# zjucsxxd/hdr2yuv

Hardware: AMD Instinct MI355X
Metric: Mpixels/s, 4K RGB->YUV420 PQ convert path (in-memory, HBM-resident) (higher is better)
Workload: dtype f32+f64

## Files before the change

### hdr2yuv_amd/api.py

```python
from __future__ import annotations

import ctypes as C
import os
import subprocess
from typing import Sequence

import numpy as np

_HERE = os.path.dirname(os.path.abspath(__file__))
_LIB = None

SAMPLE_U16, SAMPLE_F32, SAMPLE_F16 = 1, 2, 3
CHROMA_420, CHROMA_444 = 1, 3
TRANSFER_LINEAR, TRANSFER_PQ = 8, 16
MATRIX_GBR, MATRIX_BT709, MATRIX_BT2020NC, MATRIX_YDZDX, MATRIX_Y500, MATRIX_Y100 = 0, 1, 9, 11, 12, 13
MATRIX_YUVPRIME2 = 15
MATRIX_ICTCP = 14

H2Y_OK, H2Y_EINVAL, H2Y_EUNSUPPORTED, H2Y_EHIP, H2Y_ENOMEM = 0, 1, 2, 3, 4

EXPORTS = [
    "h2y_abi_version", "h2y_frame_bytes", "h2y_plane_bytes", "h2y_desc_check", "h2y_ctx_create", "h2y_ctx_destroy",
    "h2y_last_error", "h2y_ctx_set_stream", "h2y_convert_frame", "h2y_convert_batch", "h2y_convert_batch_enqueue",
    "h2y_batch_finish", "h2y_pic_stats", "h2y_matrix_convert", "h2y_subsample_420", "h2y_last_kernel_ms", "h2y_last_kernel_name", "h2y_last_kernel_variant",
    "h2y_matrix_inverse", "h2y_upsample_444", "h2y_inverse_420", "h2y_inverse_frame", "h2y_ctx_set_option", "h2y_stream_open", "h2y_stream_input", "h2y_stream_submit", "h2y_stream_output", "h2y_stream_close",
    "h2y_inverse_batch", "h2y_inverse_stream_open", "h2y_dpx_parse", "h2y_dpx_decode_batch", "h2y_dpx_stream_open",
    "h2y_tiff_parse", "h2y_tiff_layout", "h2y_tiff_decode_batch", "h2y_rgb_interleave_batch", "h2y_tiff_stream_open",
    "h2y_tiff_inverse_stream_open", "h2y_exr_parse", "h2y_exr_unpack", "h2y_exr_decode_batch", "h2y_exr_stream_open",
    "h2y_compare_batch", "h2y_stream_compare", "h2y_stream_reference", "h2y_stream_compare_result", "h2y_compare_stream_open",
    "h2y_histogram_batch", "h2y_stream_histogram", "h2y_stream_histogram_ex", "h2y_stream_histogram_result",
    "h2y_histogram_stream_open", "h2y_ssim_batch", "h2y_stream_ssim", "h2y_stream_ssim_result",
    "h2y_regions_host", "h2y_regions_batch", "h2y_stream_regions", "h2y_stream_regions_result",
    "h2y_light_batch", "h2y_stream_light", "h2y_stream_light_result",
    "h2y_lightdist_batch", "h2y_stream_lightdist", "h2y_stream_lightdist_result", "h2y_lightdist_json",
    "h2y_codelight_batch", "h2y_codelight_stream_open",
    "h2y_scenesig_batch", "h2y_codescenesig_batch", "h2y_stream_scenesig", "h2y_stream_scenesig_result", "h2y_stream_lightdist_bins",
    "h2y_scene_distance", "h2y_scene_cuts", "h2y_scene_merge", "h2y_lightdist_json_scenes",
    "h2y_linearize_batch", "h2y_pqcode_stream_open",
    "h2y_deltae_batch", "h2y_stream_deltae", "h2y_stream_deltae_result",
# ... 600 lines not shown
    L.h2y_stream_tonemap.argtypes = [C.c_void_p] + [C.c_int] * 3
    L.h2y_stream_tonemap.restype = C.c_int
    L.h2y_stream_open.argtypes = [C.c_void_p, C.POINTER(H2YDesc), C.c_int]
    L.h2y_stream_input.restype = C.c_int
    L.h2y_stream_input.argtypes = [C.c_void_p, C.POINTER(C.c_void_p)]
    L.h2y_stream_submit.restype = C.c_int
    L.h2y_stream_submit.argtypes = [C.c_void_p]
    L.h2y_stream_output.restype = C.c_int
    L.h2y_stream_output.argtypes = [C.c_void_p, C.POINTER(C.POINTER(C.c_uint16))]
    L.h2y_stream_close.restype = C.c_int
    L.h2y_stream_close.argtypes = [C.c_void_p]
    L.h2y_last_kernel_name.restype = C.c_char_p
    L.h2y_last_kernel_name.argtypes = [C.c_void_p]
    L.h2y_last_kernel_variant.restype = C.c_char_p
    L.h2y_last_kernel_variant.argtypes = [C.c_void_p]
    L.h2y_last_kernel_ms.restype = C.c_int
    L.h2y_last_kernel_ms.argtypes = [C.c_void_p, C.POINTER(C.c_float), C.POINTER(C.c_int)]
    _LIB = L
    return L


def frame_bytes(d: H2YDesc) -> int:
    return int(load_library().h2y_frame_bytes(C.byref(d)))


def desc_check(d: H2YDesc):
    why = C.c_char_p()
    rc = load_library().h2y_desc_check(C.byref(d), C.byref(why))
    return rc, (why.value or b"").decode()

# ... 1117 lines not shown
        self._stream_cmp_planes = None
        self._stream_out_words = None
        self._stream_pack_bytes = None
        self._stream_unpack_bytes = None
        self._stream_in_geom = None
        self._stream_out_geom = None
        self._stream_inverse = None
        self._stream_dpx = None
        self._stream_rgb = False

    def last_kernel_name(self) -> str:
        return (self.lib.h2y_last_kernel_name(self.h) or b"").decode()

    def last_kernel_variant(self) -> str:
        return (self.lib.h2y_last_kernel_variant(self.h) or b"").decode()
```

### hdr2yuv_amd/csrc/h2y_api.hip

```cpp
#include "h2y_shim.h"

#include <zlib.h>

static thread_local std::string g_err;

int fail(h2y_ctx *ctx, int code, const char *fmt, ...)
{
    char buf[512];
    va_list ap;
    va_start(ap, fmt);
    vsnprintf(buf, sizeof buf, fmt, ap);
    va_end(ap);
    g_err = buf;
    if (ctx) ctx->err = buf;
    return code;
}

int h2y_abi_version(void)
{
#ifdef H2Y_EXPERIMENT
    return H2Y_ABI_VERSION | H2Y_ABI_EXPERIMENT;
#else
    return H2Y_ABI_VERSION;
#endif
// ... 84 lines not shown
        HIP_TRY(ctx, hipEventCreateWithFlags(&b.ev_done, hipEventDisableTiming));
    }
    {
        std::vector<pq_recA> A(H2Y_PQ_NREC);
        std::vector<pq_recB> B(H2Y_PQ_NREC);
        pq_build_table(A.data(), B.data());
        HIP_TRY(ctx, hipMalloc(&ctx->d_table, H2Y_PQ_TABLE_BYTES));
        char *t = static_cast<char *>(ctx->d_table);
        HIP_TRY(ctx, hipMemcpy(t, A.data(), H2Y_PQ_NREC * 16, hipMemcpyHostToDevice));
        HIP_TRY(ctx, hipMemcpy(t + H2Y_PQ_NREC * 16, B.data(), H2Y_PQ_NREC * 16, hipMemcpyHostToDevice));
        {
            std::vector<pq_ext_rec> X(H2Y_PQX_NSEG);
            pq_build_table_ext(X.data());
            HIP_TRY(ctx, hipMalloc(&ctx->d_table_ext, H2Y_PQX_TABLE_BYTES));
            HIP_TRY(ctx, hipMemcpy(ctx->d_table_ext, X.data(), H2Y_PQX_TABLE_BYTES, hipMemcpyHostToDevice));
        }
        std::vector<pq_rec1> T1(H2Y_T1_NREC);
        pq_build_table1(T1.data());
        HIP_TRY(ctx, hipMalloc(&ctx->d_table1, H2Y_T1_NREC * sizeof(pq_rec1)));
        HIP_TRY(ctx, hipMemcpy(ctx->d_table1, T1.data(), H2Y_T1_NREC * sizeof(pq_rec1), hipMemcpyHostToDevice));
        HIP_TRY(ctx, hipMalloc((void **)&ctx->d_lut16, H2Y_LUT16_N * sizeof(float)));
        HIP_TRY(ctx, h2y_launch_build_lut16(ctx->stream, ctx->d_table, ctx->d_lut16));
        HIP_TRY(ctx, hipStreamSynchronize(ctx->stream));
    }
    for (batch_state &b : ctx->bs) {
        HIP_TRY(ctx, hipMalloc((void **)&b.d_assumed, 2 * sizeof(assumed_stats)));
        HIP_TRY(ctx, hipHostMalloc((void **)&b.h_assumed, 2 * sizeof(assumed_stats), hipHostMallocDefault));
        ctx->b = &b;
        const int rc = reserve_batch(ctx, 64);
        if (rc) return rc;
// ... 88 lines not shown
        (void)hipFree(b.d_partial);
        (void)hipFree(b.d_redo);
        (void)hipFree(b.d_low);
        (void)hipFree(b.d_clock);
        (void)hipHostFree(b.h_ranges);
        (void)hipHostFree(b.h_btime);
        (void)hipFree(b.d_tail);
        (void)hipFree(b.d_unit_rows);
        (void)hipHostFree(b.h_unit_rows);
        (void)hipFree(b.d_fstats);
        (void)hipHostFree(b.h_fstats);
        (void)hipFree(b.d_assumed);
        (void)hipHostFree(b.h_assumed);
    }
    (void)hipFree(ctx->d_table);
    for (void *t : ctx->d_tfn) (void)hipFree(t);
    for (int fn = 0; fn < H2Y_TFN_COUNT; fn++)
        if (ctx->d_tfn_ext[fn] && ctx->d_tfn_ext[fn] != ctx->d_table_ext) (void)hipFree(ctx->d_tfn_ext[fn]);
    (void)hipFree(ctx->d_lut16);
    (void)hipFree(ctx->d_table1);
    (void)hipFree(ctx->d_table_ext);
    (void)hipFree(ctx->d_tmp);
    (void)hipFree(ctx->d_lin);
    (void)hipFree(ctx->d_tab);
    (void)hipHostFree(ctx->h_tab);
    (void)hipFree(ctx->d_in);
    (void)hipFree(ctx->d_out);
    if (ctx->fir_stream) {
        (void)hipStreamSynchronize(ctx->fir_stream);
        (void)hipStreamDestroy(ctx->fir_stream);
// ... 1006 lines not shown
    case TIFF: return tiff_decode(ctx, tiff, clamp != 0, frames, n);
    case EXR: return exr_decode(ctx, exr, frames, n);
    default: return hipErrorInvalidValue;
    }
}

const char *decode_src::kernel() const { return kind == DPX ? "k_dpx_decode" : kind == TIFF ? "k_tiff_decode" : kind == EXR ? "k_exr_decode" : ""; }

std::string decode_src::variant() const
{
    return kind == DPX ? dpx_variant(dpx) : kind == TIFF ? tiff_variant(tiff, clamp != 0) : kind == EXR ? exr_variant(exr) : std::string();
}

const char *h2y_last_kernel_name(const h2y_ctx *ctx) { return ctx ? ctx->last_name : ""; }
const char *h2y_last_kernel_variant(const h2y_ctx *ctx) { return ctx ? ctx->last_variant.c_str() : ""; }

int h2y_last_kernel_ms(const h2y_ctx *ctx, float *ms, int *launches)
{
    if (!ctx) return H2Y_EINVAL;
    if (ms) *ms = ctx->last_ms;
    if (launches) *launches = ctx->last_launches;
    return H2Y_OK;
}
```

### hdr2yuv_amd/csrc/h2y_device.h

```cpp
#ifndef H2Y_DEVICE_H
#define H2Y_DEVICE_H

#include <hip/hip_runtime.h>
#include <stdint.h>

#include "h2y_kernels.h"
#include "h2y_math.h"

using namespace h2y;

#define WAVE 64

__device__ __forceinline__ float wave_min(float v)
{
#pragma unroll
    for (int o = 32; o > 0; o >>= 1) v = fminf(v, __shfl_xor(v, o, WAVE));
    return v;
}
__device__ __forceinline__ float wave_max(float v)
{
#pragma unroll
    for (int o = 32; o > 0; o >>= 1) v = fmaxf(v, __shfl_xor(v, o, WAVE));
    return v;
}
// ... 227 lines not shown
        const double d = pq_poly(xb, a, b);
        v = cand ? (float)d : v;
        slow = cand ? pq_ambiguous(d) : slow;
    }
    return v;
}

static __device__ __attribute__((noinline)) float tf_to_linear_careful(int cls, float v) { return tf_to_linear(cls, v); }
static __device__ __attribute__((noinline)) float tf_from_linear_careful(int cls, float v) { return tf_from_linear(cls, v); }

#define H2Y_PIPE_RUNTIME 0
#define H2Y_PIPE_PQ_IDENT 1
#define H2Y_PIPE_PQ_NORM 2
#define H2Y_PIPE_NONE 6
#define H2Y_PIPE_TFN 7

template <int PIPE> __device__ __forceinline__ float norm1(const pix_params &pp, int c, float v)
{
    const bool conv = PIPE == H2Y_PIPE_RUNTIME ? pp.convert_transfer != 0 : true;
    const bool ident = PIPE == H2Y_PIPE_RUNTIME ? pp.norm_identity : PIPE == H2Y_PIPE_PQ_IDENT;
    return (conv && !ident) ? (v - pp.offset[c]) / pp.range[c] : v;
}

template <int MODE, int PIPE>
__device__ __forceinline__ bool pixel_fast(const pix_params &pp, const pq_recA *sA, const pq_recB *sB, float G, float B, float R,
                                           uint32_t &Y, uint32_t &Cb, uint32_t &Cr)
{
    const bool conv = PIPE == H2Y_PIPE_RUNTIME ? pp.convert_transfer != 0 : true;
    float g = G, b = B, r = R;
    bool unsure = false;
// ... 164 lines not shown
```

### hdr2yuv_amd/csrc/h2y_forward.hip

```cpp
#include "h2y_shim.h"
#include "h2y_plan.h"

namespace {

const double kT1DenseShare = 0.007;
const double kFirSyncMaxFlagged = 0.004;
const int kT1SkipBatches = 32;
const int kT1SkipBatchesMax = 1024;

int tmp_depth_of(const h2y_desc *d) { return d->in_sample_type == H2Y_SAMPLE_U16 ? d->src_bit_depth : d->dst_bit_depth; }

}

void derive_params(const h2y_desc *d, pix_params *pp, bool stage_matrix_only)
{
    memset(pp, 0, sizeof *pp);
    const int tmp_depth = tmp_depth_of(d);
    const clip_limits tc = make_clip(tmp_depth, d->dst_full_range);
    const clip_limits oc = make_clip(d->dst_bit_depth, d->dst_full_range);
    pp->src_tf = tf_class(d->src_transfer);
    pp->dst_tf = tf_class(d->dst_transfer);
    if (d->src_transfer == d->dst_transfer) pp->convert_transfer = 0;
    else pp->convert_transfer = (pp->src_tf == H2Y_TF_LINEAR && pp->dst_tf == H2Y_TF_PQ) ? 1 : 2;
    pp->src_fn = pp->dst_fn = -1;
// ... 303 lines not shown
    if (r.check) b->approx_min = ident;
    firf_args fa;
    fa.frames = b->d_frames + ctx->slot_base;
    fa.n_frames = n;
    fa.width = (uint32_t)d->width;
    fa.height = (uint32_t)d->height;
    fa.wq = p.wq;
    fa.n_strips = p.strips;
    fa.n_seg = p.segments;
    fa.seg_rows = p.seg_rows;
    fa.units_per_frame = upf;
    fa.total_units = (uint32_t)p.units;
    const int fsync = ctx->opt_fir_sync >= 0 ? ctx->opt_fir_sync : (ctx->fir_flag_share > kFirSyncMaxFlagged ? 0 : 1);
    fa.sync_mask = fsync > 0 ? (uint32_t)fsync - 1u : ~0u;
    fa.table = ctx->d_table;
    fa.table1 = ctx->d_table1;
    fa.lut16 = ctx->d_lut16;
    fa.sn = r.sn;
    fa.partial = b->d_partial;
    fa.redo_count = b->d_redo;
    fa.low_flag = ident ? b->d_low : nullptr;
    fa.assumed = r.d_assumed;
    fa.pp = r.pp;
    fa.unit_rows = nullptr;
    fa.block_clock = nullptr;
    fa.mix_xcds = p.mix_xcds;
    const bool clocks = p.full && r.time_it;
    const balance bal = balance_of(ctx);
    const bool weigh = fir_weigh(p, bal, ctx->ffb_have);
    double work[8] = {0, 0, 0, 0, 0, 0, 0, 0};
// ... 115 lines not shown
        }
        a.tail_ctr = b->d_tail;
        a.tail_slices = sl.slices;
    }
    a.redo_count = t1 ? b->d_redo : nullptr;
    a.low_flag = approx ? b->d_low : nullptr;
    a.frames = b->d_frames + ctx->slot_base + f0;
    a.n_frames = nf;
    a.width = d->width;
    a.height = d->height;
    a.wq = g.wq;
    a.wq_magic = g.wq_magic;
    a.tiles_per_frame = g.tiles;
    a.chunks_per_frame = g.chunks;
    a.groups = (uint32_t)groups;
    a.table = ctx->d_table;
    a.table_src = a.table_dst = nullptr;
    a.lut16 = ctx->d_lut16;
    a.table1 = ctx->d_table1;
    a.sn = r.sn;
    a.partial = b->d_partial;
    a.assumed = r.d_assumed;
    a.pp = r.pp;
    if (r.pp.convert_transfer == 2 && !var.narrow && (var.pipe == 0 || var.pipe == 7) && (rc = set_tfn_tables(ctx, a))) return rc;
    a.tiles_magic = g.tiles > 1 ? (uint32_t)(0x100000000ull / g.tiles) : 0xFFFFFFFFu;
    const bool ev = r.time_it && b->n_ev < kMaxEvents;
    if (ev) {
        static const char *const kIn[] = {"F32", "F16", "U16"}, *const kOut[] = {"420BOX", "444", "444TMP"};
        static const char *const kPipe[] = {"RUNTIME", "PQ_IDENT", "PQ_NORM", "LUT16", "PQ_IDENT", "PQ_NORM", "NONE", "TFN"};
        const char *mode = var.mode == H2Y_MODE_YCBCR ? "YCBCR" : var.mode == H2Y_MODE_YDZDX ? "YDZDX" : var.mode == H2Y_MODE_IDENTITY ? "IDENTITY"
                         : var.mode == H2Y_MODE_YUVP2 ? "YUVP2" : "YPQRS";
// ... 455 lines not shown
    rc = ensure(ctx, ctx->b->d_partial, ctx->b->partial_cap, (size_t)grid * (h2y_fused_threads(var) / 64) * 6 * sizeof(float));
    if (rc) return rc;
    fused_args a;
    a.frames = ctx->b->d_frames;
    a.n_frames = 1;
    a.width = d->width;
    a.height = d->height;
    a.wq = g.wq;
    a.wq_magic = g.wq_magic;
    a.tiles_per_frame = g.tiles;
    a.chunks_per_frame = g.chunks;
    a.groups = 1;
    a.xcd_layout = 0;
    a.block_clock = nullptr;
    a.slice_ranges = nullptr;
    a.table = ctx->d_table;
    a.table_src = a.table_dst = nullptr;
    a.lut16 = ctx->d_lut16;
    a.table1 = ctx->d_table1;
    memset(&a.sn, 0, sizeof a.sn);
    a.tiles_magic = 0;
    a.redo_count = nullptr;
    a.low_flag = nullptr;
    a.partial = ctx->b->d_partial;
    a.assumed = ctx->b->d_assumed;
    a.pp = pp;
    HIP_TRY(ctx, h2y_launch_fused(var, grid, ctx->stream, a));
    HIP_TRY(ctx, hipStreamSynchronize(ctx->stream));
    return H2Y_OK;
}

// ... 65 lines not shown
```

### hdr2yuv_amd/csrc/h2y_kernels.h

```cpp
#ifndef H2Y_KERNELS_H
#define H2Y_KERNELS_H

#include <hip/hip_runtime.h>
#include <stdint.h>

#include "h2y_math.h"
#include "h2y_walk.h"

#ifndef H2Y_FUSED_THREADS
#define H2Y_FUSED_THREADS 512
#endif
#ifndef H2Y_FUSED_MINWAVES
#define H2Y_FUSED_MINWAVES 4
#endif

#ifndef H2Y_LOOP_THREADS
#define H2Y_LOOP_THREADS 1024
#endif

#define H2Y_LUT16_N 16384

enum { H2Y_IN_F32 = 0, H2Y_IN_F16 = 1, H2Y_IN_U16 = 2 };
enum { H2Y_OUT_420BOX = 0, H2Y_OUT_444 = 1, H2Y_OUT_444TMP = 2 };

// ... 149 lines not shown
};

struct inv_frame {
    const uint16_t *in[3];
    uint16_t *out[3];
};

#ifdef H2Y_BLOCK_TIMES
void h2y_dump_block_times(const char *path);
void h2y_dump_ff_block_times(const char *path);
#endif
int h2y_fused_threads(const fused_variant &v);
const char *h2y_fused_name(const fused_variant &v);
bool h2y_fused_grouped(const fused_variant &v);
int h2y_fused_blocks_per_cu(const fused_variant &v);
hipError_t h2y_launch_fused(const fused_variant &v, int grid, hipStream_t st, const fused_args &a);
hipError_t h2y_launch_build_lut16(hipStream_t st, const void *table, float *lut);
hipError_t h2y_launch_stats(int in_kind, int grid, hipStream_t st, const stats_args &a);
hipError_t h2y_launch_stats_final(int n_frames, hipStream_t st, const final_args &a);
hipError_t h2y_launch_fir420(hipStream_t st, const fir_args &a);
hipError_t h2y_launch_fir420_tl(hipStream_t st, const fir_args &a);
hipError_t h2y_launch_inverse(int grid, hipStream_t st, const inverse_args &a);
hipError_t h2y_launch_fir_fused(int in_kind, int mode, bool ident, bool lut16, int grid, hipStream_t st, const firf_args &a);
hipError_t h2y_launch_up444(hipStream_t st, const up_args &a);
hipError_t h2y_launch_inverse420(hipStream_t st, const inv420_args &a);
hipError_t h2y_launch_inverse420_batch(int grid, hipStream_t st, const inv420_args &base, const inv_frame *frames, int n_frames);
hipError_t h2y_launch_inverse_batch(int grid, hipStream_t st, const inverse_args &base, const inv_frame *frames, int n_frames);
int h2y_inverse420_tiles(int width, int height);
hipError_t h2y_launch_yuvp2_420(bool fir, hipStream_t st, const yuvp2_args &a);
void h2y_yuvp2_lin_table(uint16_t *lin);
// ... 338 lines not shown
```

### hdr2yuv_amd/csrc/h2y_kernels.hip

```cpp
#include <hip/hip_runtime.h>
#include <stdint.h>
#include <string.h>
#include <stdio.h>

#include "h2y_math.h"
#include "h2y_kernels.h"
#include "h2y_walk.h"
#include "h2y_device.h"

struct tile_pos {
    uint32_t tt;
    uint32_t q0, q1;
    bool row1;
};
__device__ __forceinline__ tile_pos tile_locate(uint32_t tt, uint32_t W, uint32_t H, uint32_t WQ, uint32_t magic)
{
    tile_pos t;
    uint32_t cg;
    (void)udiv_magic(tt, WQ, magic, cg);
    t.tt = tt;
    t.q0 = 2u * tt - cg;
    t.row1 = tt < WQ * (H >> 1);
    t.q1 = t.row1 ? t.q0 + WQ : t.q0;
    return t;
// ... 283 lines not shown
template <int PIPE>
__device__ __forceinline__ float pq_sample(const pix_params &pp, int c, float raw, const pq_recA *sA, const pq_recB *sB, bool &any_slow,
                                           const void *const *s_ext )
{
    if (PIPE == H2Y_PIPE_NONE) return raw;
    const float x = norm1<PIPE>(pp, c, raw);
    bool slow;
    float v = pq_fast(x, sA, sB, &slow);
    if (__builtin_expect(__builtin_amdgcn_ballot_w64(slow) != 0, 0)) {
        v = pq_ext_inline(x, v, slow, *s_ext);
        if (slow) v = pq_slow(x, *s_ext);
    }
    any_slow |= slow;
    return pix_scale(v, c == 0 ? pp.mulY : pp.mulC, c == 0 ? pp.addY : pp.addC);
}
__device__ __forceinline__ float pq_sample_rec(const pix_params &pp, int c, float x, const pq_rec &rec, bool &any_slow, const void *const *s_ext)
{
    bool sl;
    float v = pq_eval(x, rec, &sl);
    const bool zero = f2bits(x) == 0u;
    const bool slow = sl & !zero;
    bool slow2 = slow;
    v = zero ? bits2f(H2Y_PQ_AT_ZERO_BITS) : v;
    if (__builtin_expect(__builtin_amdgcn_ballot_w64(slow) != 0, 0)) {
        v = pq_ext_inline(x, v, slow2, *s_ext);
        if (slow2) v = pq_slow(x, *s_ext);
    }
    any_slow |= slow2;
    return pix_scale(v, c == 0 ? pp.mulY : pp.mulC, c == 0 ? pp.addY : pp.addC);
}
struct tfn_consts {
    uint32_t lo_base, hi_base;
    uint32_t lo_shift, hi_shift;
    uint32_t nseg_lo;
    uint32_t zero_bits, one_bits, lo_bits;
    uint32_t rho_h;
    __device__ __forceinline__ void set(int fn)
    {
        const tfn_cut c = tfn_cut_of(fn);
        lo_base = (uint32_t)(127 + c.emin) << 23;
// ... 42 lines not shown
    for (int c = 0; c < 3; c++) {
        const double v = tfn_poly(bits[c], 23 - (int)low_bits[c], ra[c], rb[c]);
        const bool zero = bits[c] == 0u, one = k.one_bits != 0u && bits[c] == 0x3F800000u;
        bool slow = pq_ambiguous(v) & !(zero | one);
        float r = zero ? bits2f(k.zero_bits) : one ? bits2f(k.one_bits) : (float)v;
        if (__builtin_expect(__builtin_amdgcn_ballot_w64(slow) != 0, 0)) {
            r = pq_ext_inline(x[c], r, slow, ext, k.lo_bits);
            if (slow) r = SRC ? tf_to_linear_careful(pp.src_tf, x0[c]) : tf_from_linear_careful(pp.dst_tf, x0[c]);
        }
        x[c] = r;
    }
}
template <int IN_KIND, int OUT_KIND, int MODE, int PIPE>
__global__ __launch_bounds__(H2Y_LOOP_THREADS) void k_fused2(fused_args a)
{
    __shared__ pq_recA s_tab[PIPE == H2Y_PIPE_NONE ? 1 : (PIPE == H2Y_PIPE_TFN ? 4 : 2) * H2Y_PQ_NREC];
    const pq_recA *sA = s_tab;
    const pq_recB *sB = reinterpret_cast<const pq_recB *>(s_tab + (PIPE == H2Y_PIPE_NONE ? 0 : H2Y_PQ_NREC));
    __shared__ uint32_t s_claim[H2Y_CLAIM_FRAMES], s_scratch[WAVE];
    __shared__ const void *s_ext;
    if (PIPE == H2Y_PIPE_TFN) {
        if (a.table_src) stage_table<H2Y_LOOP_THREADS>(a.table_src, s_tab);
        if (a.table_dst) stage_table<H2Y_LOOP_THREADS>(a.table_dst, s_tab + (PIPE == H2Y_PIPE_TFN ? 2 * H2Y_PQ_NREC : 0));
    } else if (PIPE != H2Y_PIPE_NONE) stage_table<H2Y_LOOP_THREADS>(a.table, s_tab);
    if (threadIdx.x < H2Y_CLAIM_FRAMES) s_claim[threadIdx.x] = 0u;
    if (threadIdx.x == 0) s_ext = a.pp.pq_ext;
    const pix_params pp = with_assumed(a.pp, a.assumed);
    tfn_consts k_src, k_dst;
    if (PIPE == H2Y_PIPE_TFN) {
        k_src.set(pp.src_fn > 0 ? pp.src_fn : H2Y_TFN_PQ_R);
        k_dst.set(pp.dst_fn > 0 ? pp.dst_fn : H2Y_TFN_PQ_R);
    }
    __syncthreads();

    block_clock_start(a);
    const uint32_t W = a.width, H = a.height;
    const uint32_t lane = threadIdx.x & (WAVE - 1);
    tile_in v;
    tile_pos t_cur;
// ... 51 lines not shown
#pragma unroll
                for (int col = 0; col < 4; col++) {
                    bool odd = false;
                    float g, b, r;
                    if (PIPE == H2Y_PIPE_NONE) { g = gv[col]; b = bv[col]; r = rv[col]; }
                    else if (PIPE == H2Y_PIPE_TFN) {
                        float x[3] = {norm1<H2Y_PIPE_RUNTIME>(pp, 0, gv[col]), norm1<H2Y_PIPE_RUNTIME>(pp, 1, bv[col]), norm1<H2Y_PIPE_RUNTIME>(pp, 2, rv[col])};
                        if (pp.src_fn > 0) tfn_stage3<true>(pp, k_src, s_tab, pp.tf_ext[0], x);
                        if (pp.dst_fn > 0) tfn_stage3<false>(pp, k_dst, s_tab + 2 * H2Y_PQ_NREC, pp.tf_ext[1], x);
                        odd = !(x[0] == x[0]) | !(x[1] == x[1]) | !(x[2] == x[2]);
                        g = pix_scale(x[0], pp.mulY, pp.addY);
                        b = pix_scale(x[1], pp.mulC, pp.addC);
                        r = pix_scale(x[2], pp.mulC, pp.addC);
                    } else {
                        const float xg = norm1<PIPE>(pp, 0, gv[col]), xb = norm1<PIPE>(pp, 1, bv[col]), xr = norm1<PIPE>(pp, 2, rv[col]);
                        const pq_rec cg = pq_fetch(xg, sA, sB), cb = pq_fetch(xb, sA, sB), cr = pq_fetch(xr, sA, sB);
                        __builtin_amdgcn_sched_barrier(0);
                        g = pq_sample_rec(pp, 0, xg, cg, odd, &s_ext);
                        b = pq_sample_rec(pp, 1, xb, cb, odd, &s_ext);
                        r = pq_sample_rec(pp, 2, xr, cr, odd, &s_ext);
                    }
                    bool um;
                    pix_matrix<MODE, false>(pp, g, b, r, Y[col], Cb[col], Cr[col], &um);
                    if (__builtin_expect(um | odd, 0)) pix_matrix<MODE, true>(pp, g, b, r, Y[col], Cb[col], Cr[col], &um);
                }
                row_pack<OUT_KIND, IN_KIND != H2Y_IN_U16>(pp, row, Y, Cb, Cr, o, sb, sr);
                if (row == 0) {
                    const uint32_t tt2 = ticket_resolve<H2Y_LOOP_THREADS>(n1v, deal, deal_n, s_claim, s_scratch, fo, fw.has_next(), tick, &kind, &tick2);
                    have = kind != 0;
#pragma unroll
                    for (int c = 0; c < 3; c++) src[c] = kind == 2 ? io_next.in[c] : io.in[c];
                    t2 = tile_locate(umin32(tt2 + lane, a.tiles_per_frame - 1u), W, H, a.wq, a.wq_magic);
                    IN::load4q(src[0], t2.q0, v.g0);
                    IN::load4q(src[1], t2.q0, v.b0);
                    IN::load4q(src[2], t2.q0, v.r0);
// ... 1023 lines not shown
}
const char *h2y_fused_name(const fused_variant &v)
{
    if (v.narrow) return "k_fused_narrow";
    if (v.pipe == 3) return "k_fused_lut16";
    if (v.pipe == 4 || v.pipe == 5) return "k_fused_t1";
    if (v.pipe == H2Y_PIPE_TFN) return "k_fused2";
    const bool loop_mode = v.mode == H2Y_MODE_YCBCR || v.mode == H2Y_MODE_YDZDX || (v.mode == H2Y_MODE_YUVP2 && v.out_kind == H2Y_OUT_444);
    return ((v.pipe == 1 || v.pipe == 2 || v.pipe == H2Y_PIPE_NONE) && v.even_h && loop_mode) ? "k_fused2" : "k_fused";
}
bool h2y_fused_grouped(const fused_variant &v)
{
    const char *n = h2y_fused_name(v);
    return !strcmp(n, "k_fused2") || !strcmp(n, "k_fused_t1") || !strcmp(n, "k_fused_lut16");
}
int h2y_fused_threads(const fused_variant &v)
{
    if (v.pipe == 4 || v.pipe == 5) return H2Y_T1_THREADS;
    return h2y_fused_grouped(v) ? H2Y_LOOP_THREADS : H2Y_FUSED_THREADS;
}

static fused_fn pick_fused(const fused_variant &v)
{
    if (v.pipe == 4 || v.pipe == 5)
        return v.in_kind == H2Y_IN_F16 ? pick_t1_out<H2Y_IN_F16>(v.out_kind, v.mode, v.pipe) : pick_t1_out<H2Y_IN_F32>(v.out_kind, v.mode, v.pipe);
    if (v.pipe == 3) {
        switch (v.out_kind) {
        case H2Y_OUT_420BOX: return pick_lut_mode<H2Y_OUT_420BOX>(v.mode, v.cols8);
        case H2Y_OUT_444: return pick_lut_mode<H2Y_OUT_444>(v.mode, v.cols8);
        default: return pick_lut_mode<H2Y_OUT_444TMP>(v.mode, v.cols8);
// ... 76 lines not shown
```

### hdr2yuv_amd/csrc/h2y_math.h

```cpp
#ifndef H2Y_MATH_H
#define H2Y_MATH_H

#if defined(H2Y_EXP_NOCOMPUTE) || defined(H2Y_HALF_COMPUTE) || defined(H2Y_SKIP_REDO) || defined(H2Y_EXP_NOSTATS) || defined(H2Y_EXP_NOCONFLICT) || \
    defined(H2Y_BLOCK_TIMES)
#ifndef H2Y_EXPERIMENT
#error "timing-experiment variant requested without -DH2Y_EXPERIMENT: this would build a product library with wrong bytes or debug output"
#endif
#endif

#include <stdint.h>
#include <vector>

#if defined(__HIPCC__)
#define H2Y_FN __host__ __device__ __forceinline__
#define H2Y_FN_NOINLINE __host__ __device__ inline __attribute__((noinline))
#else
#define H2Y_FN inline
#define H2Y_FN_NOINLINE inline __attribute__((noinline))
#endif

namespace h2y {

H2Y_FN uint32_t f2bits(float f) { return __builtin_bit_cast(uint32_t, f); }
H2Y_FN float bits2f(uint32_t u) { return __builtin_bit_cast(float, u); }
// ... 342 lines not shown
#else
    const uint32_t m = a > b ? a : b;
    return m > c ? m : c;
#endif
}
H2Y_FN uint32_t umin32(uint32_t a, uint32_t b)
{
#if defined(__HIP_DEVICE_COMPILE__)
    uint32_t r;
    asm("v_min_u32 %0, %1, %2" : "=v"(r) : "v"(a), "v"(b));
    return r;
#else
    return a < b ? a : b;
#endif
}
H2Y_FN uint32_t pq_rec_offset(uint32_t bits)
{
    uint32_t t = bits - (H2Y_PQ_SEG_BASE << H2Y_PQ_LOW_BITS);
    uint32_t idx = umin32(t >> H2Y_PQ_LOW_BITS, (uint32_t)H2Y_PQ_NSEG);
    return idx << 4;
}
H2Y_FN bool pq_ambiguous(double v)
{
    uint32_t lo = (uint32_t)d2bits(v);
    return ((lo << 3) + ((H2Y_PQ_AMBIG_ULPS - 0x10000000u) << 3)) < ((2u * H2Y_PQ_AMBIG_ULPS) << 3);
}

#if defined(__clang__)
typedef uint32_t u32x4 __attribute__((ext_vector_type(4)));
#else
struct alignas(16) u32x4 {
    uint32_t x, y, z, w;
};
#endif
struct pq_rec {
    u32x4 ra, rb;
};
H2Y_FN pq_rec pq_fetch(float x, const pq_recA *__restrict__ A, const pq_recB *__restrict__ B)
{
    const uint32_t off = pq_rec_offset(f2bits(x));
    pq_rec r;
    r.ra = *reinterpret_cast<const u32x4 *>(reinterpret_cast<const char *>(A) + off);
    r.rb = *reinterpret_cast<const u32x4 *>(reinterpret_cast<const char *>(B) + off);
    return r;
}
H2Y_FN float pq_eval(float x, const pq_rec &r, bool *slow)
{
    pq_recA a;
    pq_recB b;
    a.c0 = bits2d((uint64_t)r.ra.x | ((uint64_t)r.ra.y << 32));
    a.c1 = bits2d((uint64_t)r.ra.z | ((uint64_t)r.ra.w << 32));
    b.c2 = bits2d((uint64_t)r.rb.x | ((uint64_t)r.rb.y << 32));
    b.c3 = bits2f(r.rb.z);
    b.c4 = bits2f(r.rb.w);
    const double v = pq_poly(f2bits(x), a, b);
// ... 62 lines not shown
struct alignas(32) pq_ext_rec {
    pq_recA a;
    pq_recB b;
};
inline void pq_build_table_ext(pq_ext_rec *X)
{
    pq_recA *A = new pq_recA[H2Y_PQX_NSEG];
    pq_recB *B = new pq_recB[H2Y_PQX_NSEG];
    pq_build_segments(A, B, H2Y_PQX_EMIN, H2Y_PQX_NSEG);
    for (int i = 0; i < H2Y_PQX_NSEG; i++) {
        X[i].a = A[i];
        X[i].b = B[i];
    }
    delete[] A;
    delete[] B;
}
H2Y_FN bool pq_ext_try(float x, const void *ext, float *v)
{
    const uint32_t bits = f2bits(x), idx = (bits >> H2Y_PQ_LOW_BITS) - H2Y_PQX_SEG_BASE;
    if (idx >= (uint32_t)H2Y_PQX_NSEG) return false;
    const pq_ext_rec *X = reinterpret_cast<const pq_ext_rec *>(ext);
    const double d = pq_poly(bits, X[idx].a, X[idx].b);
    *v = (float)d;
    return !pq_ambiguous(d);
}

enum : int { H2Y_TFN_NONE = 0, H2Y_TFN_PQ_R = 1, H2Y_TFN_PQ_F = 2, H2Y_TFN_G24 = 3, H2Y_TFN_G24INV = 4, H2Y_TFN_RHO_R = 5, H2Y_TFN_RHO_H = 6, H2Y_TFN_COUNT = 7 };
#define H2Y_GAMMA24 ((double)2.4f)
#define H2Y_LOGF25 ((double)bits2f(0x404E0210u))

// ... 692 lines not shown
```

### hdr2yuv_amd/csrc/h2y_shim.h

```cpp
#pragma once

#include <hip/hip_runtime.h>

#include <cmath>
#include <cstdarg>
#include <cstdio>
#include <cstdlib>
#include <algorithm>
#include <cstring>
#include <memory>
#include <new>
#include <string>
#include <vector>

#include "../../include/hdr2yuv_hip.h"
#include "h2y_kernels.h"
#include "h2y_math.h"

using namespace h2y;

#pragma GCC visibility push(hidden)

struct clip_limits {
    uint32_t minCV, maxCV, minVR, maxVR, minVRC, maxVRC, Half;
// ... 164 lines not shown
    virtual int download(h2y_ctx *, int) { return H2Y_OK; }
};
enum stage_id { STAGE_UNPACK, STAGE_GAMUT, STAGE_TONEMAP, STAGE_LUT3D, STAGE_HLG, STAGE_ICTCP, STAGE_LIGHT, STAGE_LIGHTDIST, STAGE_CODELIGHT, STAGE_SCENESIG, STAGE_COMPARE, STAGE_SSIM, STAGE_DELTAE, STAGE_REGIONS, STAGE_HISTOGRAM, STAGE_SCALE, STAGE_DITHER, STAGE_PACK, STAGE_COUNT };

struct h2y_ctx {
    int device = 0;
    batch_state bs[2];
    batch_state *b = &bs[0];
    int q_head = 0, q_count = 0;
    int n_cu = 0;
    hipStream_t own_stream = nullptr, stream = nullptr;
    hipStream_t fir_stream = nullptr;
    hipEvent_t ev_fused[2] = {nullptr, nullptr}, ev_fir[2] = {nullptr, nullptr};
    bool fir_used[2] = {false, false};
    void *d_table = nullptr;
    void *d_table1 = nullptr;
    void *d_table_ext = nullptr;
    void *d_tfn[H2Y_TFN_COUNT] = {};
    void *d_tfn_ext[H2Y_TFN_COUNT] = {};
    float *d_lut16 = nullptr;
    bool bal_have = false;
    double bal_speed[8] = {1, 1, 1, 1, 1, 1, 1, 1};
    std::vector<double> bal_bspeed;
    int bal_bgrid = 0, bal_bgroups = 0;
    bool ffb_have = false;
    double ffb_speed[8] = {1, 1, 1, 1, 1, 1, 1, 1};
    int t1_skip = 0, t1_skip_len = 0;
    bool cur_skip_t1 = false;
    bool opt_t1 = true;
    bool opt_t1_steer = true;
// ... 61 lines not shown
    enum ring_kind { RING_FORWARD, RING_INVERSE, RING_PLANES } s_kind = RING_FORWARD;
    decode_src s_src;
    inv_params s_inv{};
    bool s_interleave = false;
    size_t s_pay_off = 0;
    size_t s_in_off[3] = {0, 0, 0}, s_in_bytes = 0, s_out_stride = 0;
    void *s_tab = nullptr;
    bool s_started = false;
    ring_frame s_frame;
    std::unique_ptr<ring_stage> s_stage[STAGE_COUNT];
    bool s_down = true;
    size_t s_out_bytes = 0;
    int slot_base = 0;
    float last_ms = 0.f;
    const char *last_name = "";
    std::string last_variant;
    int last_launches = 0;
    std::string err;
};

int fail(h2y_ctx *ctx, int code, const char *fmt, ...);

#define HIP_TRY(ctx, call)                                                                                  \
    do {                                                                                                    \
        hipError_t e_ = (call);                                                                             \
        if (e_ != hipSuccess) return fail(ctx, H2Y_EHIP, "%s: %s (%s:%d)", #call, hipGetErrorString(e_), __FILE__, __LINE__); \
    } while (0)

template <typename T> int ensure(h2y_ctx *ctx, T *&p, size_t &cap, size_t need_bytes)
{
// ... 141 lines not shown
```

### include/hdr2yuv_hip.h

```cpp
#ifndef HDR2YUV_HIP_H
#define HDR2YUV_HIP_H

#include <stddef.h>
#include <stdint.h>

#ifdef __cplusplus
extern "C" {
#endif

#define H2Y_ABI_VERSION 1
#define H2Y_ABI_EXPERIMENT 0x40000000


#define H2Y_SAMPLE_U16 1
#define H2Y_SAMPLE_F32 2
#define H2Y_SAMPLE_F16 3

#define H2Y_CHROMA_420 1
#define H2Y_CHROMA_444 3

#define H2Y_TRANSFER_LINEAR 8
#define H2Y_TRANSFER_PQ 16

#define H2Y_MATRIX_GBR 0
// ... 543 lines not shown
int h2y_ctx_set_chroma_siting(h2y_ctx *ctx, int chroma_sample_loc_type);

int h2y_subsample_420_sited(h2y_ctx *ctx, int width, int height, int bit_depth, int chroma_sample_loc_type, const uint16_t *d_src,
                            uint16_t *d_dst);


int h2y_ctx_set_inverse_chroma_siting(h2y_ctx *ctx, int chroma_sample_loc_type);

int h2y_upsample_444_sited(h2y_ctx *ctx, int width, int height, int chroma_sample_loc_type, unsigned min_cv, unsigned max_cv,
                           const uint16_t *d_src, uint16_t *d_dst);

int h2y_last_kernel_ms(const h2y_ctx *ctx, float *ms, int *launches);

const char *h2y_last_kernel_name(const h2y_ctx *ctx);
const char *h2y_last_kernel_variant(const h2y_ctx *ctx);

#ifdef __cplusplus
}
#endif
#endif
```

Baseline: 373,300.

## Stage deeper PQ table in LDS for k_fused2 to cover small inputs

```diff
diff --git a/hdr2yuv_amd/api.py b/hdr2yuv_amd/api.py
--- a/hdr2yuv_amd/api.py
+++ b/hdr2yuv_amd/api.py
@@ -22,7 +22,7 @@
 EXPORTS = [
     "h2y_abi_version", "h2y_frame_bytes", "h2y_plane_bytes", "h2y_desc_check", "h2y_ctx_create", "h2y_ctx_destroy",
     "h2y_last_error", "h2y_ctx_set_stream", "h2y_convert_frame", "h2y_convert_batch", "h2y_convert_batch_enqueue",
-    "h2y_batch_finish", "h2y_pic_stats", "h2y_matrix_convert", "h2y_subsample_420", "h2y_last_kernel_ms", "h2y_last_kernel_name", "h2y_last_kernel_variant",
+    "h2y_batch_finish", "h2y_pic_stats", "h2y_matrix_convert", "h2y_subsample_420", "h2y_last_kernel_ms", "h2y_last_kernel_name", "h2y_last_kernel_variant", "h2y_last_kernel_pq_lds_emin",
     "h2y_matrix_inverse", "h2y_upsample_444", "h2y_inverse_420", "h2y_inverse_frame", "h2y_ctx_set_option", "h2y_stream_open", "h2y_stream_input", "h2y_stream_submit", "h2y_stream_output", "h2y_stream_close",
     "h2y_inverse_batch", "h2y_inverse_stream_open", "h2y_dpx_parse", "h2y_dpx_decode_batch", "h2y_dpx_stream_open",
     "h2y_tiff_parse", "h2y_tiff_layout", "h2y_tiff_decode_batch", "h2y_rgb_interleave_batch", "h2y_tiff_stream_open",
@@ -653,6 +653,8 @@
     L.h2y_last_kernel_name.argtypes = [C.c_void_p]
     L.h2y_last_kernel_variant.restype = C.c_char_p
     L.h2y_last_kernel_variant.argtypes = [C.c_void_p]
+    L.h2y_last_kernel_pq_lds_emin.restype = C.c_int
+    L.h2y_last_kernel_pq_lds_emin.argtypes = [C.c_void_p]
     L.h2y_last_kernel_ms.restype = C.c_int
     L.h2y_last_kernel_ms.argtypes = [C.c_void_p, C.POINTER(C.c_float), C.POINTER(C.c_int)]
     _LIB = L
@@ -1800,3 +1802,6 @@
 
     def last_kernel_variant(self) -> str:
         return (self.lib.h2y_last_kernel_variant(self.h) or b"").decode()
+
+    def last_kernel_pq_lds_emin(self) -> int:
+        return int(self.lib.h2y_last_kernel_pq_lds_emin(self.h))
diff --git a/hdr2yuv_amd/csrc/h2y_api.hip b/hdr2yuv_amd/csrc/h2y_api.hip
--- a/hdr2yuv_amd/csrc/h2y_api.hip
+++ b/hdr2yuv_amd/csrc/h2y_api.hip
@@ -122,6 +122,13 @@
             pq_build_table_ext(X.data());
             HIP_TRY(ctx, hipMalloc(&ctx->d_table_ext, H2Y_PQX_TABLE_BYTES));
             HIP_TRY(ctx, hipMemcpy(ctx->d_table_ext, X.data(), H2Y_PQX_TABLE_BYTES, hipMemcpyHostToDevice));
+            std::vector<pq_recA> A2(H2Y_PQ2_NREC);
+            std::vector<pq_recB> B2(H2Y_PQ2_NREC);
+            pq_build_table_deep(A2.data(), B2.data(), A.data(), B.data(), X.data());
+            HIP_TRY(ctx, hipMalloc(&ctx->d_table_deep, H2Y_PQ2_TABLE_BYTES));
+            char *t2 = static_cast<char *>(ctx->d_table_deep);
+            HIP_TRY(ctx, hipMemcpy(t2, A2.data(), H2Y_PQ2_NREC * 16, hipMemcpyHostToDevice));
+            HIP_TRY(ctx, hipMemcpy(t2 + H2Y_PQ2_NREC * 16, B2.data(), H2Y_PQ2_NREC * 16, hipMemcpyHostToDevice));
         }
         std::vector<pq_rec1> T1(H2Y_T1_NREC);
         pq_build_table1(T1.data());
@@ -240,6 +247,7 @@
         (void)hipHostFree(b.h_assumed);
     }
     (void)hipFree(ctx->d_table);
+    (void)hipFree(ctx->d_table_deep);
     for (void *t : ctx->d_tfn) (void)hipFree(t);
     for (int fn = 0; fn < H2Y_TFN_COUNT; fn++)
         if (ctx->d_tfn_ext[fn] && ctx->d_tfn_ext[fn] != ctx->d_table_ext) (void)hipFree(ctx->d_tfn_ext[fn]);
@@ -1276,6 +1284,7 @@
 
 const char *h2y_last_kernel_name(const h2y_ctx *ctx) { return ctx ? ctx->last_name : ""; }
 const char *h2y_last_kernel_variant(const h2y_ctx *ctx) { return ctx ? ctx->last_variant.c_str() : ""; }
+int h2y_last_kernel_pq_lds_emin(const h2y_ctx *ctx) { return ctx ? ctx->last_table_emin : 0; }
 
 int h2y_last_kernel_ms(const h2y_ctx *ctx, float *ms, int *launches)
 {
diff --git a/hdr2yuv_amd/csrc/h2y_device.h b/hdr2yuv_amd/csrc/h2y_device.h
--- a/hdr2yuv_amd/csrc/h2y_device.h
+++ b/hdr2yuv_amd/csrc/h2y_device.h
@@ -265,6 +265,7 @@
 #define H2Y_PIPE_PQ_NORM 2
 #define H2Y_PIPE_NONE 6
 #define H2Y_PIPE_TFN 7
+#define H2Y_FUSED2_DEEP(PIPE) ((PIPE) == H2Y_PIPE_PQ_IDENT || (PIPE) == H2Y_PIPE_PQ_NORM)
 
 template <int PIPE> __device__ __forceinline__ float norm1(const pix_params &pp, int c, float v)
 {
diff --git a/hdr2yuv_amd/csrc/h2y_forward.hip b/hdr2yuv_amd/csrc/h2y_forward.hip
--- a/hdr2yuv_amd/csrc/h2y_forward.hip
+++ b/hdr2yuv_amd/csrc/h2y_forward.hip
@@ -341,6 +341,7 @@
     const int fsync = ctx->opt_fir_sync >= 0 ? ctx->opt_fir_sync : (ctx->fir_flag_share > kFirSyncMaxFlagged ? 0 : 1);
     fa.sync_mask = fsync > 0 ? (uint32_t)fsync - 1u : ~0u;
     fa.table = ctx->d_table;
+    ctx->last_table_emin = H2Y_PQ_EMIN;
     fa.table1 = ctx->d_table1;
     fa.lut16 = ctx->d_lut16;
     fa.sn = r.sn;
@@ -486,7 +487,9 @@
     a.tiles_per_frame = g.tiles;
     a.chunks_per_frame = g.chunks;
     a.groups = (uint32_t)groups;
-    a.table = ctx->d_table;
+    const int table_emin = h2y_fused_table_emin(var);
+    a.table = table_emin == H2Y_PQ2_EMIN ? ctx->d_table_deep : ctx->d_table;
+    ctx->last_table_emin = table_emin;
     a.table_src = a.table_dst = nullptr;
     a.lut16 = ctx->d_lut16;
     a.table1 = ctx->d_table1;
@@ -972,7 +975,8 @@
     a.xcd_layout = 0;
     a.block_clock = nullptr;
     a.slice_ranges = nullptr;
-    a.table = ctx->d_table;
+    ctx->last_table_emin = h2y_fused_table_emin(var);
+    a.table = ctx->last_table_emin == H2Y_PQ2_EMIN ? ctx->d_table_deep : ctx->d_table;
     a.table_src = a.table_dst = nullptr;
     a.lut16 = ctx->d_lut16;
     a.table1 = ctx->d_table1;
diff --git a/hdr2yuv_amd/csrc/h2y_kernels.h b/hdr2yuv_amd/csrc/h2y_kernels.h
--- a/hdr2yuv_amd/csrc/h2y_kernels.h
+++ b/hdr2yuv_amd/csrc/h2y_kernels.h
@@ -187,6 +187,7 @@
 const char *h2y_fused_name(const fused_variant &v);
 bool h2y_fused_grouped(const fused_variant &v);
 int h2y_fused_blocks_per_cu(const fused_variant &v);
+int h2y_fused_table_emin(const fused_variant &v);
 hipError_t h2y_launch_fused(const fused_variant &v, int grid, hipStream_t st, const fused_args &a);
 hipError_t h2y_launch_build_lut16(hipStream_t st, const void *table, float *lut);
 hipError_t h2y_launch_stats(int in_kind, int grid, hipStream_t st, const stats_args &a);
diff --git a/hdr2yuv_amd/csrc/h2y_kernels.hip b/hdr2yuv_amd/csrc/h2y_kernels.hip
--- a/hdr2yuv_amd/csrc/h2y_kernels.hip
+++ b/hdr2yuv_amd/csrc/h2y_kernels.hip
@@ -321,6 +321,7 @@
     any_slow |= slow;
     return pix_scale(v, c == 0 ? pp.mulY : pp.mulC, c == 0 ? pp.addY : pp.addC);
 }
+template <int EMIN>
 __device__ __forceinline__ float pq_sample_rec(const pix_params &pp, int c, float x, const pq_rec &rec, bool &any_slow, const void *const *s_ext)
 {
     bool sl;
@@ -330,7 +331,7 @@
     bool slow2 = slow;
     v = zero ? bits2f(H2Y_PQ_AT_ZERO_BITS) : v;
     if (__builtin_expect(__builtin_amdgcn_ballot_w64(slow) != 0, 0)) {
-        v = pq_ext_inline(x, v, slow2, *s_ext);
+        v = pq_ext_inline(x, v, slow2, *s_ext, (uint32_t)(127 + EMIN) << 23);
         if (slow2) v = pq_slow(x, *s_ext);
     }
     any_slow |= slow2;
@@ -403,15 +404,16 @@
 template <int IN_KIND, int OUT_KIND, int MODE, int PIPE>
 __global__ __launch_bounds__(H2Y_LOOP_THREADS) void k_fused2(fused_args a)
 {
-    __shared__ pq_recA s_tab[PIPE == H2Y_PIPE_NONE ? 1 : (PIPE == H2Y_PIPE_TFN ? 4 : 2) * H2Y_PQ_NREC];
+    constexpr int EMIN = H2Y_FUSED2_DEEP(PIPE) ? H2Y_PQ2_EMIN : H2Y_PQ_EMIN, NREC = H2Y_PQ_NREC_OF(EMIN);
+    __shared__ pq_recA s_tab[PIPE == H2Y_PIPE_NONE ? 1 : (PIPE == H2Y_PIPE_TFN ? 4 : 2) * NREC];
     const pq_recA *sA = s_tab;
-    const pq_recB *sB = reinterpret_cast<const pq_recB *>(s_tab + (PIPE == H2Y_PIPE_NONE ? 0 : H2Y_PQ_NREC));
+    const pq_recB *sB = reinterpret_cast<const pq_recB *>(s_tab + (PIPE == H2Y_PIPE_NONE ? 0 : NREC));
     __shared__ uint32_t s_claim[H2Y_CLAIM_FRAMES], s_scratch[WAVE];
     __shared__ const void *s_ext;
     if (PIPE == H2Y_PIPE_TFN) {
         if (a.table_src) stage_table<H2Y_LOOP_THREADS>(a.table_src, s_tab);
         if (a.table_dst) stage_table<H2Y_LOOP_THREADS>(a.table_dst, s_tab + (PIPE == H2Y_PIPE_TFN ? 2 * H2Y_PQ_NREC : 0));
-    } else if (PIPE != H2Y_PIPE_NONE) stage_table<H2Y_LOOP_THREADS>(a.table, s_tab);
+    } else if (PIPE != H2Y_PIPE_NONE) stage16<H2Y_LOOP_THREADS, 2 * NREC>(a.table, s_tab);
     if (threadIdx.x < H2Y_CLAIM_FRAMES) s_claim[threadIdx.x] = 0u;
     if (threadIdx.x == 0) s_ext = a.pp.pq_ext;
     const pix_params pp = with_assumed(a.pp, a.assumed);
@@ -493,11 +495,11 @@
                         r = pix_scale(x[2], pp.mulC, pp.addC);
                     } else {
                         const float xg = norm1<PIPE>(pp, 0, gv[col]), xb = norm1<PIPE>(pp, 1, bv[col]), xr = norm1<PIPE>(pp, 2, rv[col]);
-                        const pq_rec cg = pq_fetch(xg, sA, sB), cb = pq_fetch(xb, sA, sB), cr = pq_fetch(xr, sA, sB);
+                        const pq_rec cg = pq_fetch<EMIN>(xg, sA, sB), cb = pq_fetch<EMIN>(xb, sA, sB), cr = pq_fetch<EMIN>(xr, sA, sB);
                         __builtin_amdgcn_sched_barrier(0);
-                        g = pq_sample_rec(pp, 0, xg, cg, odd, &s_ext);
-                        b = pq_sample_rec(pp, 1, xb, cb, odd, &s_ext);
-                        r = pq_sample_rec(pp, 2, xr, cr, odd, &s_ext);
+                        g = pq_sample_rec<EMIN>(pp, 0, xg, cg, odd, &s_ext);
+                        b = pq_sample_rec<EMIN>(pp, 1, xb, cb, odd, &s_ext);
+                        r = pq_sample_rec<EMIN>(pp, 2, xr, cr, odd, &s_ext);
                     }
                     bool um;
                     pix_matrix<MODE, false>(pp, g, b, r, Y[col], Cb[col], Cr[col], &um);
@@ -1551,6 +1553,10 @@
     const char *n = h2y_fused_name(v);
     return !strcmp(n, "k_fused2") || !strcmp(n, "k_fused_t1") || !strcmp(n, "k_fused_lut16");
 }
+int h2y_fused_table_emin(const fused_variant &v)
+{
+    return H2Y_FUSED2_DEEP(v.pipe) && !v.narrow && !strcmp(h2y_fused_name(v), "k_fused2") ? H2Y_PQ2_EMIN : H2Y_PQ_EMIN;
+}
 int h2y_fused_threads(const fused_variant &v)
 {
     if (v.pipe == 4 || v.pipe == 5) return H2Y_T1_THREADS;
diff --git a/hdr2yuv_amd/csrc/h2y_math.h b/hdr2yuv_amd/csrc/h2y_math.h
--- a/hdr2yuv_amd/csrc/h2y_math.h
+++ b/hdr2yuv_amd/csrc/h2y_math.h
@@ -380,10 +380,12 @@
     return a < b ? a : b;
 #endif
 }
-H2Y_FN uint32_t pq_rec_offset(uint32_t bits)
-{
-    uint32_t t = bits - (H2Y_PQ_SEG_BASE << H2Y_PQ_LOW_BITS);
-    uint32_t idx = umin32(t >> H2Y_PQ_LOW_BITS, (uint32_t)H2Y_PQ_NSEG);
+#define H2Y_PQ_NSEG_OF(EMIN) ((1 - (EMIN)) * H2Y_PQ_SEG_PER_BINADE)
+#define H2Y_PQ_NREC_OF(EMIN) (H2Y_PQ_NSEG_OF(EMIN) + 1)
+template <int EMIN = H2Y_PQ_EMIN> H2Y_FN uint32_t pq_rec_offset(uint32_t bits)
+{
+    uint32_t t = bits - ((uint32_t)(127 + EMIN) << 23);
+    uint32_t idx = umin32(t >> H2Y_PQ_LOW_BITS, (uint32_t)H2Y_PQ_NSEG_OF(EMIN));
     return idx << 4;
 }
 H2Y_FN bool pq_ambiguous(double v)
@@ -402,9 +404,9 @@
 struct pq_rec {
     u32x4 ra, rb;
 };
-H2Y_FN pq_rec pq_fetch(float x, const pq_recA *__restrict__ A, const pq_recB *__restrict__ B)
-{
-    const uint32_t off = pq_rec_offset(f2bits(x));
+template <int EMIN = H2Y_PQ_EMIN> H2Y_FN pq_rec pq_fetch(float x, const pq_recA *__restrict__ A, const pq_recB *__restrict__ B)
+{
+    const uint32_t off = pq_rec_offset<EMIN>(f2bits(x));
     pq_rec r;
     r.ra = *reinterpret_cast<const u32x4 *>(reinterpret_cast<const char *>(A) + off);
     r.rb = *reinterpret_cast<const u32x4 *>(reinterpret_cast<const char *>(B) + off);
@@ -497,6 +499,22 @@
     }
     delete[] A;
     delete[] B;
+}
+#define H2Y_PQ2_EMIN (-62)
+#define H2Y_PQ2_NSEG H2Y_PQ_NSEG_OF(H2Y_PQ2_EMIN)
+#define H2Y_PQ2_NREC H2Y_PQ_NREC_OF(H2Y_PQ2_EMIN)
+#define H2Y_PQ2_TABLE_BYTES (H2Y_PQ2_NREC * 32)
+inline void pq_build_table_deep(pq_recA *A, pq_recB *B, const pq_recA *A25, const pq_recB *B25, const pq_ext_rec *X)
+{
+    const int below = H2Y_PQ2_NSEG - H2Y_PQ_NSEG, x0 = (H2Y_PQ2_EMIN - H2Y_PQX_EMIN) * H2Y_PQ_SEG_PER_BINADE;
+    for (int i = 0; i < below; i++) {
+        A[i] = X[x0 + i].a;
+        B[i] = X[x0 + i].b;
+    }
+    for (int i = 0; i < H2Y_PQ_NREC; i++) {
+        A[below + i] = A25[i];
+        B[below + i] = B25[i];
+    }
 }
 H2Y_FN bool pq_ext_try(float x, const void *ext, float *v)
 {
diff --git a/hdr2yuv_amd/csrc/h2y_shim.h b/hdr2yuv_amd/csrc/h2y_shim.h
--- a/hdr2yuv_amd/csrc/h2y_shim.h
+++ b/hdr2yuv_amd/csrc/h2y_shim.h
@@ -202,6 +202,7 @@
     hipEvent_t ev_fused[2] = {nullptr, nullptr}, ev_fir[2] = {nullptr, nullptr};
     bool fir_used[2] = {false, false};
     void *d_table = nullptr;
+    void *d_table_deep = nullptr;
     void *d_table1 = nullptr;
     void *d_table_ext = nullptr;
     void *d_tfn[H2Y_TFN_COUNT] = {};
@@ -293,6 +294,7 @@
     int slot_base = 0;
     float last_ms = 0.f;
     const char *last_name = "";
+    int last_table_emin = 0;
     std::string last_variant;
     int last_launches = 0;
     std::string err;
diff --git a/include/hdr2yuv_hip.h b/include/hdr2yuv_hip.h
--- a/include/hdr2yuv_hip.h
+++ b/include/hdr2yuv_hip.h
@@ -581,6 +581,7 @@
 
 const char *h2y_last_kernel_name(const h2y_ctx *ctx);
 const char *h2y_last_kernel_variant(const h2y_ctx *ctx);
+int h2y_last_kernel_pq_lds_emin(const h2y_ctx *ctx);
 
 #ifdef __cplusplus
 }
```

After: 376,200 (median of 4 runs). About the same (+0.8%).
